# cassiePython/NeRF-Art

Hardware: AMD Instinct MI355X
Metric: rays/sec at 480x270x128spp VolSDF render (higher is better)
Workload: dtype pixels bf16x3 (sdf, nabla, radiance, compositing of the 192 final samples: f32 split into 2 bf16 terms, 3 MFMAs per product, f32 accumulate), Algorithm-1 sampler fp16x1 on error-compensated one-term weights (fp16 act x fp16 weight, 1 MFMA per product, f32 accumulate; model.calibrate_sampler()), guar

## Files before the change

### nerfart_amd/build.py

```python
from __future__ import annotations

import os
import shutil
import subprocess
import sys

CSRC = os.path.join(os.path.dirname(os.path.abspath(__file__)), "csrc")
LIB = os.path.join(CSRC, "libnerfart_hip.so")
PUBLIC_HEADER = os.path.join(os.path.dirname(os.path.dirname(CSRC)), "include", "nerfart_hip.h")
SOURCES = ["capi_common.cpp", "wgrad.hip", "pass2_operands.hip", "render_backward.hip", "mlp_chain.hip", "mlp_chain_bf16.hip", "mlp_chain_f16x2.hip", "mlp_chain_f16x1.hip", "mlp_k2_w32.hip", "mlp_grad_bf16.hip", "mlp_backward_bf16.hip", "volsdf_render.hip", "volsdf_backward.hip", "neus_render.hip", "raygen.hip", "clip_vit.hip", "style_heads.hip", "ray_casting.hip", "vgg_conv.hip", "pack_blob.hip", "geo_feature.hip", "marching_cubes.hip"]
HEADERS = ["nerfart_common.h", "host_util.h", "ray_common.h", "mlp_common.h", "mlp_bf16_core.h", "gemm_f16.h", "gemm_f32.h", "mc_table.h"]
INCLUDES = {"mlp_chain_f16x2.hip": ["mlp_chain_bf16.hip", "mlp_grad_bf16.hip"], "mlp_chain_f16x1.hip": ["mlp_chain_bf16.hip"]}
FLAGS = ["--offload-arch=gfx950", "-O3", "-std=c++17", "-fPIC", "-fno-slp-vectorize", "-x", "hip"]
VARIANTS = {"scan_generic": ("volsdf_render.hip", ["-DNERFART_SCAN_GENERIC"])}


def variant_lib(name: str) -> str:
    return os.path.join(CSRC, f"libnerfart_hip_{name}.so")


def _hipcc() -> str:
    for c in (os.environ.get("HIPCC"), shutil.which("hipcc"), "/opt/rocm/bin/hipcc"):
        if c and os.path.exists(c):
            return c
    raise RuntimeError("hipcc not found (need ROCm with gfx950 support)")


def _stale(target: str, deps) -> bool:
    if not os.path.exists(target):
        return True
    t = os.path.getmtime(target)
    return any(os.path.getmtime(d) > t for d in deps)


def build(verbose: bool = True, force: bool = False) -> str:
    hipcc = _hipcc()
    bdir = os.path.join(CSRC, "_build")
    os.makedirs(bdir, exist_ok=True)
    hdrs = [os.path.join(CSRC, h) for h in HEADERS] + [PUBLIC_HEADER]
    objs = []
    for s in SOURCES:
        src = os.path.join(CSRC, s)
        if not os.path.exists(src):
            continue
        obj = os.path.join(bdir, os.path.splitext(s)[0] + ".o")
        deps = [src] + hdrs + [os.path.join(CSRC, i) for i in INCLUDES.get(s, [])]
        if force or _stale(obj, deps):
            cmd = [hipcc] + FLAGS + ["-c", src, "-o", obj]
            if verbose:
                print("[nerfart build]", " ".join(cmd), flush=True)
            subprocess.check_call(cmd)
        objs.append(obj)
    if force or _stale(LIB, objs):
        cmd = [hipcc, "--offload-arch=gfx950", "-shared", "-fPIC", "-o", LIB] + objs
        if verbose:
            print("[nerfart build]", " ".join(cmd), flush=True)
        subprocess.check_call(cmd)
    for name, (src_name, defs) in VARIANTS.items():
        src = os.path.join(CSRC, src_name)
        obj = os.path.join(bdir, os.path.splitext(src_name)[0] + f".{name}.o")
        if force or _stale(obj, [src] + hdrs):
            cmd = [hipcc] + FLAGS + defs + ["-c", src, "-o", obj]
            if verbose:
                print("[nerfart build]", " ".join(cmd), flush=True)
            subprocess.check_call(cmd)
        vlib = variant_lib(name)
        others = [o for o in objs if os.path.basename(o) != os.path.splitext(src_name)[0] + ".o"]
        if force or _stale(vlib, others + [obj]):
            cmd = [hipcc, "--offload-arch=gfx950", "-shared", "-fPIC", "-o", vlib] + others + [obj]
            if verbose:
                print("[nerfart build]", " ".join(cmd), flush=True)
            subprocess.check_call(cmd)
    return LIB


if __name__ == "__main__":
    print(build(force="--force" in sys.argv))
```

### nerfart_amd/csrc/mlp_chain_f16x1.hip

```cpp
#define NERFART_F16X2 1
#define NERFART_F16X1 1
#define NERFART_K2_ONLY 1
#define b16 f16x1
#define sdf_bf16_v1 sdf_f16x1
#include "mlp_chain_bf16.hip"
```

Baseline: 308,900.

## Add hand-scheduled SDF-only f16x1 sampler kernel with interleaved LDS reads and epilogues

Adds a new SDF-only kernel for the fp16x1 sampler path. It software-pipelines LDS weight reads, MFMA issue with explicit lgkmcnt waits, global weight streaming and the previous layer's activation epilogue inside one compile-time unrolled schedule. It uses single-term MFMAs for hidden layers and two-term MFMAs only for the encoding layers. The previous implementation is kept as a reference and can be selected with an environment variable. The hand-written asm and exact wait counts are fragile, and wrong counts could cause hazards or incorrect results.

Result: faster. 332,900 (median of 6 runs) (+7.8%).

```diff
diff --git a/nerfart_amd/build.py b/nerfart_amd/build.py
--- a/nerfart_amd/build.py
+++ b/nerfart_amd/build.py
@@ -8,7 +8,7 @@
 CSRC = os.path.join(os.path.dirname(os.path.abspath(__file__)), "csrc")
 LIB = os.path.join(CSRC, "libnerfart_hip.so")
 PUBLIC_HEADER = os.path.join(os.path.dirname(os.path.dirname(CSRC)), "include", "nerfart_hip.h")
-SOURCES = ["capi_common.cpp", "wgrad.hip", "pass2_operands.hip", "render_backward.hip", "mlp_chain.hip", "mlp_chain_bf16.hip", "mlp_chain_f16x2.hip", "mlp_chain_f16x1.hip", "mlp_k2_w32.hip", "mlp_grad_bf16.hip", "mlp_backward_bf16.hip", "volsdf_render.hip", "volsdf_backward.hip", "neus_render.hip", "raygen.hip", "clip_vit.hip", "style_heads.hip", "ray_casting.hip", "vgg_conv.hip", "pack_blob.hip", "geo_feature.hip", "marching_cubes.hip"]
+SOURCES = ["capi_common.cpp", "wgrad.hip", "pass2_operands.hip", "render_backward.hip", "mlp_chain.hip", "mlp_chain_bf16.hip", "mlp_chain_f16x2.hip", "mlp_chain_f16x1.hip", "mlp_k2_f16x1_to.hip", "mlp_k2_w32.hip", "mlp_grad_bf16.hip", "mlp_backward_bf16.hip", "volsdf_render.hip", "volsdf_backward.hip", "neus_render.hip", "raygen.hip", "clip_vit.hip", "style_heads.hip", "ray_casting.hip", "vgg_conv.hip", "pack_blob.hip", "geo_feature.hip", "marching_cubes.hip"]
 HEADERS = ["nerfart_common.h", "host_util.h", "ray_common.h", "mlp_common.h", "mlp_bf16_core.h", "gemm_f16.h", "gemm_f32.h", "mc_table.h"]
 INCLUDES = {"mlp_chain_f16x2.hip": ["mlp_chain_bf16.hip", "mlp_grad_bf16.hip"], "mlp_chain_f16x1.hip": ["mlp_chain_bf16.hip"]}
 FLAGS = ["--offload-arch=gfx950", "-O3", "-std=c++17", "-fPIC", "-fno-slp-vectorize", "-x", "hip"]
diff --git a/nerfart_amd/csrc/mlp_chain_f16x1.hip b/nerfart_amd/csrc/mlp_chain_f16x1.hip
--- a/nerfart_amd/csrc/mlp_chain_f16x1.hip
+++ b/nerfart_amd/csrc/mlp_chain_f16x1.hip
@@ -2,5 +2,5 @@
 #define NERFART_F16X1 1
 #define NERFART_K2_ONLY 1
 #define b16 f16x1
-#define sdf_bf16_v1 sdf_f16x1
+#define sdf_bf16_v1 sdf_f16x1_ref
 #include "mlp_chain_bf16.hip"
diff --git a/nerfart_amd/csrc/mlp_k2_f16x1_to.hip b/nerfart_amd/csrc/mlp_k2_f16x1_to.hip
--- /dev/null
+++ b/nerfart_amd/csrc/mlp_k2_f16x1_to.hip
@@ -0,0 +1,317 @@
+#define NERFART_F16X2 1
+#define NERFART_F16X1 1
+#define NERFART_K2_ONLY 1
+#define b16 f16x1
+#include "mlp_bf16_core.h"
+#include <cstdlib>
+
+namespace nerfart {
+namespace f16x1 {
+
+struct ToState {
+    u32x4 cur[2][8], nxt[2][8];
+    f32x4 acc[2][2][2];
+    Unit enc[2][2];
+    f32x4 bt[2], rw[2];
+    Work2 w;
+    float dot[2];
+    u32x4 rh[3], rl[3];
+    unsigned addr, baddr;
+};
+
+template <int KIND, bool TAIL>
+struct ToCfg {
+    static constexpr int NKS = KIND == 0 ? 8 : (KIND == 1 ? 9 : 2), NH = KIND == 0 ? 8 : (KIND == 1 ? 7 : 0);
+    static constexpr int NI = 2 * NKS, PPC = KIND == 2 ? 8 : 2, N = NI * PPC;
+    static constexpr bool full(int ci) { return ci >= 0 && ci < N && ((ci % NI) >> 1) >= NH; }
+    static constexpr int nfr(int ci) { return (ci >= 0 && ci < N) ? (full(ci) ? 2 : 1) : 0; }
+    static constexpr int auxn(int P) { return TAIL ? (P == 7 ? 2 : 4) : 2; }
+    static constexpr int naux(int ci, int P0) { return (ci >= 0 && ci < N && (ci % NI) == NI - 4) ? auxn(P0 + ci / NI) : 0; }
+    static constexpr int hi_off(int ci) {
+        const int pl = ci / NI, u = (ci % NI) >> 1, t = ci & 1;
+        if (KIND == 2) return (16 * u + 2 * pl + t) * 2048;
+        if (u < 8) return (4 * u + 2 * pl + t) * 2048;
+        return (2 * pl + t) * 2048 + 1024;
+    }
+    static constexpr int lo_off(int ci) {
+        const int pl = ci / NI, u = (ci % NI) >> 1, t = ci & 1;
+        if (KIND == 1 && u == 8) return (4 + 2 * pl + t) * 2048 + 1024;
+        return hi_off(ci) + 1024;
+    }
+};
+
+template <int OFFH, int OFFL>
+__device__ __forceinline__ void to_read_2(u32x4& fh, u32x4& fl, unsigned addr) {
+    asm volatile("ds_read_b128 %0, %2 offset:%3\n\tds_read_b128 %1, %2 offset:%4" : "=&v"(fh), "=&v"(fl) : "v"(addr), "i"(OFFH), "i"(OFFL));
+}
+template <int OFF>
+__device__ __forceinline__ void to_read_f(f32x4& v, unsigned addr) {
+    asm volatile("ds_read_b128 %0, %1 offset:%2" : "=&v"(v) : "v"(addr), "i"(OFF));
+}
+
+template <int CNT, bool PAD, bool FULL>
+__device__ __forceinline__ void to_wait_mfma(const u32x4 ah, const u32x4 al, const u32x4 b0h, const u32x4 b0l, const u32x4 b1h, const u32x4 b1l,
+                                             f32x4& a0, f32x4& a1) {
+    if constexpr (FULL) {
+        if constexpr (PAD) {
+            asm volatile("s_waitcnt lgkmcnt(%8)\n\t"
+                         "s_nop 1\n\t"
+                         "v_mfma_f32_16x16x32_f16 %0, %2, %4, %0\n\t"
+                         "v_mfma_f32_16x16x32_f16 %1, %2, %6, %1\n\t"
+                         "v_mfma_f32_16x16x32_f16 %0, %2, %5, %0\n\t"
+                         "v_mfma_f32_16x16x32_f16 %1, %2, %7, %1\n\t"
+                         "v_mfma_f32_16x16x32_f16 %0, %3, %4, %0\n\t"
+                         "v_mfma_f32_16x16x32_f16 %1, %3, %6, %1"
+                         : "+v"(a0), "+v"(a1) : "v"(ah), "v"(al), "v"(b0h), "v"(b0l), "v"(b1h), "v"(b1l), "i"(CNT));
+        } else {
+            asm volatile("s_waitcnt lgkmcnt(%8)\n\t"
+                         "v_mfma_f32_16x16x32_f16 %0, %2, %4, %0\n\t"
+                         "v_mfma_f32_16x16x32_f16 %1, %2, %6, %1\n\t"
+                         "v_mfma_f32_16x16x32_f16 %0, %2, %5, %0\n\t"
+                         "v_mfma_f32_16x16x32_f16 %1, %2, %7, %1\n\t"
+                         "v_mfma_f32_16x16x32_f16 %0, %3, %4, %0\n\t"
+                         "v_mfma_f32_16x16x32_f16 %1, %3, %6, %1"
+                         : "+v"(a0), "+v"(a1) : "v"(ah), "v"(al), "v"(b0h), "v"(b0l), "v"(b1h), "v"(b1l), "i"(CNT));
+        }
+    } else if constexpr (PAD) {
+        asm volatile("s_waitcnt lgkmcnt(%5)\n\t"
+                     "s_nop 1\n\t"
+                     "v_mfma_f32_16x16x32_f16 %0, %2, %3, %0\n\t"
+                     "v_mfma_f32_16x16x32_f16 %1, %2, %4, %1"
+                     : "+v"(a0), "+v"(a1) : "v"(ah), "v"(b0h), "v"(b1h), "i"(CNT));
+    } else {
+        asm volatile("s_waitcnt lgkmcnt(%5)\n\t"
+                     "v_mfma_f32_16x16x32_f16 %0, %2, %3, %0\n\t"
+                     "v_mfma_f32_16x16x32_f16 %1, %2, %4, %1"
+                     : "+v"(a0), "+v"(a1) : "v"(ah), "v"(b0h), "v"(b1h), "i"(CNT));
+    }
+}
+
+template <int NXT>
+__device__ __forceinline__ unsigned to_acquire(Stream& s, Stream& sx, int base, int q, bool next_skip) {
+    wait_glds();
+    __syncthreads();
+    const unsigned cur = lds_addr(s.lds + s.pb * CHUNK_FLOATS), dst = lds_addr(s.lds + (s.pb ^ 1) * CHUNK_FLOATS);
+    const int w = wave_id();
+    s.iss_dst = dst + w * 8192;
+    if constexpr (NXT == 2) {
+        s.iss_src = s.blob + base + w * 2048;
+        sx.iss_src = s.iss_src; sx.iss_dst = s.iss_dst; sx.lo_exec = ~0ull;
+    } else {
+        s.iss_src = s.blob + base + (w * 16 + 4 * q) * 512;
+        if constexpr (NXT != 0) {
+            const float* s8 = s.blob + base + (8 * 16 + 4 * q) * 512;
+            sx.iss_src = (w == 7) ? s.iss_src : ((w == 0) ? s8 - 256 : s8);
+            sx.iss_dst = (w == 7) ? s.iss_dst : ((w == 0) ? dst : dst + 8192);
+            const bool on = (NXT == 1 || next_skip) && (w == 7 || w < 2);
+            sx.lo_exec = __builtin_amdgcn_readfirstlane((int)on) != 0 ? ~0ull : 0ull;
+        }
+    }
+    s.pb ^= 1;
+    return cur;
+}
+
+template <int KIND, bool TAIL, int NXT, int PL, int P, int I>
+struct ToItems {
+    using C = ToCfg<KIND, TAIL>;
+    static __device__ __forceinline__ void run(ToState& st, const Stream& s, const Stream& sx) {
+        if constexpr (I < C::NI) {
+            constexpr int ci = PL * C::NI + I, u = I >> 1, t = I & 1, pp = P & 1, S = ci % 3, S2 = (ci + 2) % 3, P0 = P - PL;
+            constexpr bool FULL = C::full(ci);
+            constexpr int PENDING = C::nfr(ci + 1) + C::naux(ci - 2, P0) + C::naux(ci - 1, P0);
+            if constexpr (KIND == 2 || (KIND == 1 && u >= 7)) {
+                constexpr int q = KIND == 2 ? u : u - 7;
+                to_wait_mfma<PENDING, I == 0, true>(st.rh[S], st.rl[S], st.enc[0][q].h, st.enc[0][q].l, st.enc[1][q].h, st.enc[1][q].l,
+                                                    st.acc[pp][t][0], st.acc[pp][t][1]);
+            } else {
+                to_wait_mfma<PENDING, I == 0, false>(st.rh[S], st.rh[S], st.cur[0][u], st.cur[0][u], st.cur[1][u], st.cur[1][u],
+                                                     st.acc[pp][t][0], st.acc[pp][t][1]);
+            }
+            static_assert(FULL == (KIND == 2 || (KIND == 1 && u >= 7)), "three-term k-steps");
+            if constexpr (ci + 2 < C::N) {
+                if constexpr (C::full(ci + 2)) to_read_2<C::hi_off(ci + 2), C::lo_off(ci + 2)>(st.rh[S2], st.rl[S2], st.addr);
+                else lds_read_hi<C::hi_off(ci + 2)>(st.rh[S2], st.addr);
+            }
+            constexpr bool BIAS = !(TAIL && P == 7);
+            if constexpr (I == C::NI - 4) {
+                constexpr int pn = (P + 1) & 7, boff = (P == 7 ? 1024 : 0) + 2 * pn * 64;
+                if constexpr (BIAS) { to_read_f<boff>(st.bt[0], st.baddr); to_read_f<boff + 64>(st.bt[1], st.baddr); }
+                if constexpr (TAIL) { to_read_f<1024 + 2 * P * 64>(st.rw[0], st.baddr); to_read_f<1024 + 2 * P * 64 + 64>(st.rw[1], st.baddr); }
+            }
+            if constexpr (KIND == 2) {
+                if constexpr (P == 0) stream_piece<2 * I>(s);
+            } else {
+                constexpr bool ODD = NXT != 0;
+                if constexpr (I == 0) stream_piece<4 * PL>(s);
+                if constexpr (I == 13) { stream_piece<4 * PL + 2>(s); if constexpr (ODD) stream_piece<4 * PL + 1>(sx); }
+                if constexpr (I == 15) { if constexpr (ODD) stream_piece<4 * PL + 3>(sx); }
+            }
+            constexpr int HOST = TAIL ? (P == 0 ? 1 : 2) : ((KIND != 0 && P == 0) ? 0 : 1);
+            if constexpr (HOST == 1 && KIND == 2) {
+                constexpr int pr = I, tt = pr >> 1, r0 = 2 * (pr & 1);
+                unsigned h0 = 0, l0 = 0, h1 = 0, l1 = 0, dout = 0;
+                epi_phase<0, 0>(st.acc[pp ^ 1][tt][0][r0], st.acc[pp ^ 1][tt][0][r0 + 1], st.w, h0, l0, 0.f, true, 0u, dout);
+                epi_phase<0, 0>(st.acc[pp ^ 1][tt][1][r0], st.acc[pp ^ 1][tt][1][r0 + 1], st.w.b, h1, l1, 0.f, true, 0u, dout);
+                epi_phase<0, 1>(st.acc[pp ^ 1][tt][0][r0], st.acc[pp ^ 1][tt][0][r0 + 1], st.w, h0, l0, 0.f, true, 0u, dout);
+                epi_phase<0, 1>(st.acc[pp ^ 1][tt][1][r0], st.acc[pp ^ 1][tt][1][r0 + 1], st.w.b, h1, l1, 0.f, true, 0u, dout);
+                epi_phase<0, 2>(0.f, 0.f, st.w, h0, l0, 0.f, true, 0u, dout);
+                epi_phase<0, 2>(0.f, 0.f, st.w.b, h1, l1, 0.f, true, 0u, dout);
+                st.nxt[0][P - 1][pr] = h0;
+                st.nxt[1][P - 1][pr] = h1;
+            }
+            if constexpr (HOST == 1 && KIND != 2 && I >= 1 && I <= 12) {
+                constexpr int pr = (I - 1) / 3, ph = (I - 1) % 3, tt = pr >> 1, r0 = 2 * (pr & 1);
+                unsigned h0 = 0, l0 = 0, h1 = 0, l1 = 0, dout = 0;
+                epi_phase<0, ph>(st.acc[pp ^ 1][tt][0][r0], st.acc[pp ^ 1][tt][0][r0 + 1], st.w, h0, l0, 0.f, true, 0u, dout);
+                epi_phase<0, ph>(st.acc[pp ^ 1][tt][1][r0], st.acc[pp ^ 1][tt][1][r0 + 1], st.w.b, h1, l1, 0.f, true, 0u, dout);
+                if constexpr (ph == 2) {
+                    if constexpr (P == 0) { st.cur[0][7][pr] = h0; st.cur[1][7][pr] = h1; }
+                    else { st.nxt[0][P - 1][pr] = h0; st.nxt[1][P - 1][pr] = h1; }
+                }
+            }
+            if constexpr (HOST == 2 && I >= 1 && I <= 8) {
+                constexpr int tt = (I - 1) >> 2, r = (I - 1) & 3;
+#pragma unroll
+                for (int gp = 0; gp < 2; ++gp) {
+                    const float a = st.acc[pp ^ 1][tt][gp][r];
+                    const float y = fmaxf(a, 0.f) + __builtin_amdgcn_logf(1.0f + __builtin_amdgcn_exp2f(-fabsf(a)));
+                    st.dot[gp] = fmaf(y, st.rw[tt][r], st.dot[gp]);
+                }
+            }
+            if constexpr (I == C::NI - 1) {
+                if constexpr (BIAS) {
+                    asm volatile("" : "+v"(st.bt[0]), "+v"(st.bt[1]));
+                    st.acc[pp ^ 1][0][0] = st.bt[0]; st.acc[pp ^ 1][0][1] = st.bt[0];
+                    st.acc[pp ^ 1][1][0] = st.bt[1]; st.acc[pp ^ 1][1][1] = st.bt[1];
+                }
+                if constexpr (TAIL) asm volatile("" : "+v"(st.rw[0]), "+v"(st.rw[1]));
+            }
+            __builtin_amdgcn_sched_barrier(0);
+            ToItems<KIND, TAIL, NXT, PL, P, I + 1>::run(st, s, sx);
+        }
+    }
+};
+
+template <int KIND, bool TAIL, int NXT, int Q>
+__device__ __forceinline__ void to_chunk(ToState& st, Stream& s, Stream& sx, int base, int q, bool next_skip) {
+    using C = ToCfg<KIND, TAIL>;
+    st.addr = to_acquire<NXT>(s, sx, base, q, next_skip) + lane_id() * 16;
+    asm volatile("s_waitcnt lgkmcnt(0)" ::: "memory");
+    if constexpr (C::full(0)) {
+        to_read_2<C::hi_off(0), C::lo_off(0)>(st.rh[0], st.rl[0], st.addr);
+        to_read_2<C::hi_off(1), C::lo_off(1)>(st.rh[1], st.rl[1], st.addr);
+    } else {
+        lds_read_hi<C::hi_off(0)>(st.rh[0], st.addr);
+        lds_read_hi<C::hi_off(1)>(st.rh[1], st.addr);
+    }
+    if constexpr (KIND == 2) {
+        ToItems<2, false, NXT, 0, 0, 0>::run(st, s, sx); ToItems<2, false, NXT, 1, 1, 0>::run(st, s, sx);
+        ToItems<2, false, NXT, 2, 2, 0>::run(st, s, sx); ToItems<2, false, NXT, 3, 3, 0>::run(st, s, sx);
+        ToItems<2, false, NXT, 4, 4, 0>::run(st, s, sx); ToItems<2, false, NXT, 5, 5, 0>::run(st, s, sx);
+        ToItems<2, false, NXT, 6, 6, 0>::run(st, s, sx); ToItems<2, false, NXT, 7, 7, 0>::run(st, s, sx);
+    } else {
+        ToItems<KIND, TAIL, NXT, 0, 2 * Q, 0>::run(st, s, sx);
+        ToItems<KIND, TAIL, NXT, 1, 2 * Q + 1, 0>::run(st, s, sx);
+    }
+}
+
+__device__ __forceinline__ int to_first_chunk(int l) { return l == 0 ? 0 : (l <= 4 ? 4 * l - 3 : 4 * l - 2); }
+
+__global__ void __launch_bounds__(WG_THREADS, 2)
+k_sdf_only_to(const float* __restrict__ blob, PointSrc src, float R_bg, float* __restrict__ sdf_out, int out_stride) {
+    extern __shared__ __attribute__((aligned(16))) float smem[];
+    const int* hdr = reinterpret_cast<const int*>(blob);
+    float* aux = smem + 2 * CHUNK_FLOATS;
+    const int lane = lane_id(), g = lane >> 4, j = lane & 15, wv = wave_id();
+    load_aux(aux, blob, hdr, SURF_AUX_FLOATS);
+    const unsigned ntiles = (src.M + 255u) / 256u;
+    if (blockIdx.x >= ntiles) return;
+    Stream s = make_stream(blob, aux, smem, hdr[2]);
+    stream_start(s);
+    Stream sx = s;
+    const int base0 = __builtin_amdgcn_readfirstlane(s.tab[0]);
+    const unsigned bl = lds_addr(aux) + g * 16;
+    ToState st;
+    for (unsigned tile = blockIdx.x; tile < ntiles; tile += gridDim.x) {
+        Pt pt[2];
+#pragma unroll
+        for (int gp = 0; gp < 2; ++gp) {
+            pt[gp] = fetch_point(src, tile * 256u + wv * 32 + gp * 16 + j, false);
+            encode_units(pt[gp].x, pt[gp].y, pt[gp].z, g, -1, st.enc[gp]);
+        }
+        st.dot[0] = 0.f; st.dot[1] = 0.f;
+        st.w = {};
+#pragma unroll
+        for (int t = 0; t < 2; ++t) {
+            const f32x4 b = *reinterpret_cast<const f32x4*>(aux + 16 * t + 4 * g);
+            st.acc[0][t][0] = b; st.acc[0][t][1] = b;
+        }
+        st.baddr = bl;
+        to_chunk<2, false, 0, 0>(st, s, sx, __builtin_amdgcn_readfirstlane(s.tab[1]), 0, false);
+#pragma unroll
+        for (int u = 0; u < 7; ++u) { st.cur[0][u] = st.nxt[0][u]; st.cur[1][u] = st.nxt[1][u]; }
+#pragma nounroll
+        for (int L = 1; L < 7; ++L) {
+            const int bL = __builtin_amdgcn_readfirstlane(s.tab[to_first_chunk(L)]), bN = __builtin_amdgcn_readfirstlane(s.tab[to_first_chunk(L + 1)]);
+            st.baddr = bl + L * 1024;
+            if (L == 4) {
+                to_chunk<1, false, 1, 0>(st, s, sx, bL, 1, false);
+                to_chunk<1, false, 1, 1>(st, s, sx, bL, 2, false);
+                to_chunk<1, false, 1, 2>(st, s, sx, bL, 3, false);
+                to_chunk<1, false, 0, 3>(st, s, sx, bN, 0, false);
+            } else {
+                to_chunk<0, false, 0, 0>(st, s, sx, bL, 1, false);
+                to_chunk<0, false, 0, 1>(st, s, sx, bL, 2, false);
+                to_chunk<0, false, 0, 2>(st, s, sx, bL, 3, false);
+                to_chunk<0, false, 3, 3>(st, s, sx, bN, 0, L == 3);
+            }
+#pragma unroll
+            for (int u = 0; u < 7; ++u) { st.cur[0][u] = st.nxt[0][u]; st.cur[1][u] = st.nxt[1][u]; }
+        }
+        {
+            const int b7 = __builtin_amdgcn_readfirstlane(s.tab[to_first_chunk(7)]);
+            st.baddr = bl + 7 * 1024;
+            to_chunk<0, true, 0, 0>(st, s, sx, b7, 1, false);
+            to_chunk<0, true, 0, 1>(st, s, sx, b7, 2, false);
+            to_chunk<0, true, 0, 2>(st, s, sx, b7, 3, false);
+            to_chunk<0, true, 2, 3>(st, s, sx, base0, 0, false);
+        }
+        asm volatile("s_nop 7\n\ts_nop 7" ::: "memory");
+#pragma unroll
+        for (int tt = 0; tt < 2; ++tt)
+#pragma unroll
+            for (int r = 0; r < 4; ++r)
+#pragma unroll
+                for (int gp = 0; gp < 2; ++gp) {
+                    const float a = st.acc[1][tt][gp][r];
+                    const float y = fmaxf(a, 0.f) + __builtin_amdgcn_logf(1.0f + __builtin_amdgcn_exp2f(-fabsf(a)));
+                    st.dot[gp] = fmaf(y, st.rw[tt][r], st.dot[gp]);
+                }
+#pragma unroll
+        for (int gp = 0; gp < 2; ++gp) {
+            const unsigned m = tile * 256u + wv * 32 + gp * 16 + j;
+            float sdf = sum_over_groups(st.dot[gp]) + aux[SURF_AUX_B8];
+            if (R_bg > 0.f) sdf = fminf(sdf, R_bg - sqrtf(fmaf(pt[gp].z, pt[gp].z, fmaf(pt[gp].y, pt[gp].y, pt[gp].x * pt[gp].x))));
+            if (g == 0 && m < src.M) {
+                if (src.pts) sdf_out[m] = sdf;
+                else {
+                    const unsigned slot = m / (unsigned)src.n_per_ray;
+                    sdf_out[(size_t)slot * out_stride + (m - slot * (unsigned)src.n_per_ray)] = sdf;
+                }
+            }
+        }
+    }
+    wait_glds();
+}
+
+}
+
+int sdf_f16x1_ref(const float* blob, const PointSrc& s, float R_bg, float* out, int out_stride, hipStream_t st);
+
+int sdf_f16x1(const float* blob, const PointSrc& s, float R_bg, float* out, int out_stride, hipStream_t st) {
+    const char* e = std::getenv("NERFART_K2_F16X1");
+    if (e != nullptr && e[0] == 'r') return sdf_f16x1_ref(blob, s, R_bg, out, out_stride, st);
+    return f16x1::launch_chain(0, (long long)s.M, f16x1::k_sdf_only_to, (s.M + 255u) / 256u, st, blob, s, R_bg, out, out_stride);
+}
+
+}
```
